# kyprifog/ballista

Measured on AMD Instinct MI355X. Metric: tpch_q1_sf100_rows_per_sec, higher is better.
Workload: dtype f64; 1 GPU; TPC-H Q1 SF100 (scan+filter+group-by aggregate), 600037902 lineitem rows resident in HBM, Arrow layout, Int32 order keys; lineitem_rows=600037902, rows_per_gpu=600037902, partitioning=1 GPU, whole tables

## Files before the change

ballista_amd/csrc/host/sop.cpp:

```cpp
#include "sop.hpp"

#include <cmath>
#include <cstring>
#include <limits>

namespace bhip {

namespace {

struct Builder {
    const Schema& schema;
    SopPlan& out;
    Builder(const Schema& s, SopPlan& o) : schema(s), out(o) {}

    int column(int schema_idx) {
        for (size_t i = 0; i < out.col_map.size(); ++i)
            if (out.col_map[i] == schema_idx) return (int)i;
        if ((int)out.col_map.size() >= SOP_NCOL) return -1;
        out.col_map.push_back(schema_idx);
        return (int)out.col_map.size() - 1;
    }

    int plain_column(const ExprPtr& e) const {
        if (e->kind != BHIP_EXPR_COLUMN) return -1;
        return schema.index_of(e->name);
    }

    bool predicate(const ExprPtr& e) {
        if (e->kind == BHIP_EXPR_BINARY && e->name == "And") return predicate(e->args[0]) && predicate(e->args[1]);
        if (e->kind != BHIP_EXPR_BINARY) return false;
        static const char* ops[] = {"Eq", "Lt", "LtEq", "Gt", "GtEq"};
        static const int flipped[] = {0, 3, 4, 1, 2};
        int k = -1;
        for (int i = 0; i < 5; ++i)
            if (e->name == ops[i]) k = i;
        if (k < 0) return false;
        ExprPtr colside = e->args[0], litside = e->args[1];
        if (colside->kind == BHIP_EXPR_LITERAL) { std::swap(colside, litside); k = flipped[k]; }
        const int ci = plain_column(colside);
        if (ci < 0) return false;
        const int t = schema.fields[ci].dtype;
        if (litside->kind != BHIP_EXPR_LITERAL || litside->is_null || litside->dtype != t) return false;
        double lit;
        bool is_int;
        if (t == DT_FLOAT64) { lit = litside->f64; is_int = false; }
        else if (t == DT_INT32 || t == DT_DATE32) { lit = (double)litside->i64; is_int = true; }
        else return false;
        if (std::isnan(lit)) return false;
        const double inf = std::numeric_limits<double>::infinity();
        double lo = -inf, hi = inf;
        switch (k) {
            case 0: lo = hi = lit; break;
            case 1: hi = is_int ? lit - 1.0 : std::nextafter(lit, -inf); break;
            case 2: hi = lit; break;
            case 3: lo = is_int ? lit + 1.0 : std::nextafter(lit, inf); break;
            default: lo = lit; break;
        }
        const int c = column(ci);
        if (c < 0) return false;
        for (int i = 0; i < out.prog.n_ranges; ++i)
            if (out.prog.ranges[i].col == c) {
                if (lo > out.prog.ranges[i].lo) out.prog.ranges[i].lo = lo;
                if (hi < out.prog.ranges[i].hi) out.prog.ranges[i].hi = hi;
                return true;
            }
        if (out.prog.n_ranges >= SOP_NRANGE) return false;
        SopRange& r = out.prog.ranges[out.prog.n_ranges++];
        memset(&r, 0, sizeof(r));
        r.col = (uint8_t)c;
        r.is32 = is_int ? 1 : 0;
        r.lo = lo;
        r.hi = hi;
        return true;
    }

    struct Factor { bool has_col; bool is32; int schema_col; double sgn, add; std::string text; };

    bool f64_column(const ExprPtr& e, int& col, bool& is32) const {
        if (e->kind == BHIP_EXPR_CAST && e->dtype == DT_FLOAT64) {
            const int i = plain_column(e->args[0]);
            if (i < 0) return false;
            const int t = schema.fields[i].dtype;
            if (t != DT_INT32 && t != DT_DATE32) return false;
            col = i; is32 = true;
            return true;
        }
        const int i = plain_column(e);
        if (i < 0 || schema.fields[i].dtype != DT_FLOAT64) return false;
        col = i; is32 = false;
        return true;
    }

    static bool f64_literal(const ExprPtr& e, double& v) {
        if (e->kind != BHIP_EXPR_LITERAL || e->dtype != DT_FLOAT64 || e->is_null) return false;
        v = e->f64;
        return true;
    }

    bool factor(const ExprPtr& e, Factor& f) const {
        f.text = e->to_string();
        f.has_col = true; f.is32 = false; f.schema_col = -1; f.sgn = 1.0; f.add = -0.0;
        double lit;
        if (f64_literal(e, lit)) { f.has_col = false; f.sgn = 0.0; f.add = lit; return true; }
        if (f64_column(e, f.schema_col, f.is32)) return true;
        if (e->kind == BHIP_EXPR_BINARY && (e->name == "Plus" || e->name == "Minus")) {
            const bool plus = e->name == "Plus";
            if (f64_literal(e->args[0], lit) && f64_column(e->args[1], f.schema_col, f.is32)) {
                f.sgn = plus ? 1.0 : -1.0;
                f.add = lit;
                return true;
            }
            if (f64_literal(e->args[1], lit) && f64_column(e->args[0], f.schema_col, f.is32)) {
                f.sgn = 1.0;
                f.add = plus ? lit : -lit;
                return true;
            }
        }
        return false;
    }

    bool chain(const ExprPtr& e, std::vector<Factor>& fs) const {
        Factor f;
        if (factor(e, f)) { fs.push_back(f); return true; }
        if (e->kind == BHIP_EXPR_BINARY && e->name == "Multiply") {
            if (!chain(e->args[0], fs)) return false;
            if (!factor(e->args[1], f)) return false;
            fs.push_back(f);
            return true;
        }
        return false;
    }
};

}

bool build_sop(const Schema& schema, const ExprPtr& predicate, const std::vector<ExprPtr>& keys,
               const std::vector<SopAccExpr>& accs, SopPlan& out) {
    memset(&out.prog, 0, sizeof(out.prog));
    out.col_map.clear();
    out.key_info.clear();
    Builder b(schema, out);
    if (predicate && !b.predicate(predicate)) return false;
    for (int i = 0; i < out.prog.n_ranges; ++i)
        if (out.prog.ranges[i].lo > out.prog.ranges[i].hi) return false;
    if (keys.size() > (size_t)SOP_NKEY) return false;
    for (size_t i = 0; i < keys.size(); ++i) {
        const int si = b.plain_column(keys[i]);
        if (si < 0) return false;
        const int t = schema.fields[si].dtype;
        int kind, width;
        if (t == DT_INT32 || t == DT_DATE32) { kind = SOP_KEY_I32; width = 4; }
        else if (t == DT_INT64 || t == DT_UINT64) { kind = SOP_KEY_I64; width = 8; }
        else if (t == DT_UTF8) { kind = SOP_KEY_UTF8; width = 8; }
        else return false;
        if (keys.size() == 3 && i >= 1 && kind != SOP_KEY_I32) return false;
        const int c = b.column(si);
        if (c < 0) return false;
        SopKey& k = out.prog.keys[out.prog.n_keys++];
        k.col = (uint8_t)c;
        k.kind = (uint8_t)kind;
        k.pad[0] = k.pad[1] = 0;
        const int pos = i == 0 ? 0 : (i == 1 ? 8 : 12);
        out.key_info.push_back(ProgramBuilder::KeyInfo{pos, width, 0, t});
    }
    std::vector<std::string> last_chain;
    for (size_t a = 0; a < accs.size(); ++a) {
        if (accs[a].kind != ACC_SUM_F64) return false;
        std::vector<Builder::Factor> fs;
        if (!b.chain(accs[a].expr, fs)) return false;
        size_t common = 0;
        if (!last_chain.empty() && fs.size() > last_chain.size()) {
            common = last_chain.size();
            for (size_t i = 0; i < last_chain.size(); ++i)
                if (fs[i].text != last_chain[i]) { common = 0; break; }
        }
        for (size_t i = common; i < fs.size(); ++i) {
            if (out.prog.n_steps >= SOP_NSTEP) return false;
            SopStep& st = out.prog.steps[out.prog.n_steps++];
            memset(&st, 0, sizeof(st));
            st.has_col = fs[i].has_col ? 1 : 0;
            st.is32 = fs[i].is32 ? 1 : 0;
            st.start = i == 0 ? 1 : 0;
            st.acc = 0xFF;
            st.sgn = fs[i].sgn;
            st.add = fs[i].add;
            if (fs[i].has_col) {
                const int c = b.column(fs[i].schema_col);
                if (c < 0) return false;
                st.col = (uint8_t)c;
            }
        }
        out.prog.steps[out.prog.n_steps - 1].acc = (uint8_t)a;
        last_chain.clear();
        for (auto& f : fs) last_chain.push_back(f.text);
    }
    out.prog.n_cols = (int)out.col_map.size();
    return true;
}

bool sop_columns_bindable(const SopPlan& plan, const Batch& b, bool range_nulls_ok) {
    for (size_t i = 0; i < plan.col_map.size(); ++i) {
        if (!b.cols[plan.col_map[i]].validity) continue;
        bool ranged = false;
        for (int r = 0; r < plan.prog.n_ranges; ++r) ranged = ranged || plan.prog.ranges[r].col == (uint8_t)i;
        if (!(range_nulls_ok && ranged)) return false;
    }
    return true;
}

void bind_sop(SopPlan& plan, const Batch& b) {
    plan.prog.n_rows = b.n_rows;
    for (size_t i = 0; i < plan.col_map.size(); ++i) {
        const Column& c = b.cols[plan.col_map[i]];
        SopColumn& sc = plan.prog.cols[i];
        sc.data = c.data ? c.data->ptr() : nullptr;
        sc.offsets = c.offsets ? c.offsets->as<int32_t>() : nullptr;
        sc.validity = c.validity ? c.validity->as<uint64_t>() : nullptr;
        sc.dtype = c.dtype;
        sc.data_bytes = (int32_t)c.data_bytes;
        sc.width = c.utf8_width(b.n_rows);
        sc.pad = 0;
    }
}

bool lean_eligible(const SopProgram& prog) {
    if (prog.n_keys > 2) return false;
    for (int q = 0; q < prog.n_keys; ++q)
        if (prog.keys[q].kind != SOP_KEY_I32 && prog.keys[q].kind != SOP_KEY_UTF8) return false;
    for (int s = 0; s < prog.n_steps; ++s) {
        const SopStep& st = prog.steps[s];
        if (!st.has_col || st.is32) return false;
        if (st.sgn != 1.0 && st.sgn != -1.0) return false;
    }
    return true;
}

bool lean_bindable(const SopPlan& plan, const Batch& b) {
    for (int ci : plan.col_map) {
        const Column& c = b.cols[ci];
        if (c.data && ((uintptr_t)c.data->ptr() & 15)) return false;
        if (c.offsets && ((uintptr_t)c.offsets->ptr() & 15)) return false;
        if (c.dtype == DT_UTF8 && c.data && !c.data->owned()) return false;
    }
    return true;
}

}
```

ballista_amd/csrc/lean_kernel.h:

```cpp
#pragma once
#include <hip/hip_runtime.h>
#include "kernels.h"
#include "launch_common.h"
#include "reduce_device.h"
#include "sop.h"
#include "vm_device.h"

namespace bhip {

#ifndef LEAN_U_VALUE
#define LEAN_U_VALUE 2
#endif
constexpr int LEAN_U = LEAN_U_VALUE;
constexpr int LEAN_SUB = BLOCK * 2;
constexpr int LEAN_TILE = LEAN_SUB * LEAN_U;
constexpr int LEAN_ROWS = 2 * LEAN_U;
constexpr uint32_t LEAN_MAX_STR = 3;

template <int GMAX, int NSTEP>
struct LeanLds {
    static constexpr int NG = GMAX > 1 ? GMAX : 0;
    double acc[NG * NSTEP * BLOCK + 1];
    uint32_t cnt[NG * BLOCK + 1];
    uint64_t keys[AGG_GMAX];
    uint32_t ng, lock, overflow, pad;
    uint64_t red[4][GMAX * NSTEP];
    uint64_t rowred[4][GMAX];
    uint64_t rowtot[GMAX];
};

struct LeanU3 { uint32_t a, b, c; };
struct alignas(8) LeanU2 { uint32_t x, y; };
struct alignas(16) LeanU4 { uint32_t x, y, z, w; };

__device__ inline LeanU2 lean_ld2(const BHIP_GLOBAL char* p) {
    const BHIP_GLOBAL LeanU2* q = (const BHIP_GLOBAL LeanU2*)p;
    LeanU2 v;
    v.x = q->x; v.y = q->y;
    return v;
}
__device__ inline LeanU4 lean_ld4(const BHIP_GLOBAL char* p) {
    const BHIP_GLOBAL LeanU4* q = (const BHIP_GLOBAL LeanU4*)p;
    LeanU4 v;
    v.x = q->x; v.y = q->y; v.z = q->z; v.w = q->w;
    return v;
}

__device__ inline uint64_t lean_uniform_u64(uint64_t v) {
    const uint32_t lo = __builtin_amdgcn_readfirstlane((uint32_t)v), hi = __builtin_amdgcn_readfirstlane((uint32_t)(v >> 32));
    return ((uint64_t)hi << 32) | lo;
}

__device__ inline uint32_t lean_str_word(uint32_t raw, uint32_t len) {
    return (__builtin_amdgcn_ubfe(raw, 0u, len << 3) << 8) | len;
}

template <bool ON>
struct LeanLens {
    uint32_t any[2] = {0u, 0u};
    uint32_t all[2] = {~0u, ~0u};
    __device__ void see(int q, uint32_t len) { any[q] |= len; all[q] &= len; }
};
template <>
struct LeanLens<false> {
    uint32_t bad = 0;
    __device__ void see(int, uint32_t len) { bad |= len; }
};

template <int GMAX, int NSTEP>
struct LeanKeyTable {
    int ng_c = 0;
    uint64_t gk[GMAX];
    __device__ LeanKeyTable() {
#pragma unroll
        for (int g = 0; g < GMAX; ++g) gk[g] = 0;
    }
    __device__ bool lookup(LeanLds<GMAX, NSTEP>& lds, int lane, const uint64_t (&key)[LEAN_ROWS], const bool (&live)[LEAN_ROWS],
                           int (&lg)[LEAN_ROWS]) {
        if constexpr (GMAX == 1) {
#pragma unroll
            for (int r = 0; r < LEAN_ROWS; ++r) lg[r] = live[r] ? 0 : -1;
            return true;
        } else {
            volatile uint32_t* v_ng = &lds.ng;
            volatile uint32_t* v_over = &lds.overflow;
            for (;;) {
                bool pending = false;
#pragma unroll
                for (int r = 0; r < LEAN_ROWS; ++r) {
                    int found = -2;
#pragma unroll
                    for (int g2 = 0; g2 < GMAX; ++g2) found = (g2 < ng_c && key[r] == gk[g2]) ? g2 : found;
                    lg[r] = live[r] ? found : -1;
                    pending |= (lg[r] == -2);
                }
                const uint64_t pmask = __ballot(pending);
                if (__builtin_expect(pmask == 0, 1)) return true;
                if (__builtin_amdgcn_readfirstlane(*v_over)) return false;
                if (__builtin_amdgcn_readfirstlane(*v_ng) == (uint32_t)ng_c) {
                    if (lane == (int)__builtin_ctzll(pmask)) {
                        uint64_t mine = 0;
#pragma unroll
                        for (int r = LEAN_ROWS - 1; r >= 0; --r)
                            if (lg[r] == -2) mine = key[r];
                        while (atomicCAS(&lds.lock, 0u, 1u) != 0u) {}
                        const int n2 = (int)*v_ng;
                        bool have = false;
                        for (int g2 = 0; g2 < n2; ++g2) have |= (lds.keys[g2] == mine);
                        if (!have) {
                            if (n2 < GMAX) {
                                lds.keys[n2] = mine;
                                __threadfence_block();
                                *v_ng = (uint32_t)(n2 + 1);
                            } else {
                                *v_over = 1;
                            }
                        }
                        __threadfence_block();
                        atomicExch(&lds.lock, 0u);
                    }
                }
                ng_c = __builtin_amdgcn_readfirstlane((int)*v_ng);
#pragma unroll
                for (int g2 = 0; g2 < GMAX; ++g2) gk[g2] = lean_uniform_u64(lds.keys[g2]);
            }
        }
    }
};

template <int GMAX, int NSTEP, int NRANGE, class Lens, class Lookup, class Accumulate>
__device__ inline bool lean_tail(const SopProgram& S, int64_t tail0, int64_t n_rows, Lens& lens, Lookup&& lookup,
                                 Accumulate&& accumulate) {
    constexpr int NKEY = 2;
    const int tid = threadIdx.x;
    for (int k = 0; k < LEAN_TILE / BLOCK; ++k) {
        const int64_t i = tail0 + (int64_t)k * BLOCK + tid;
        const bool in = i < n_rows;
        bool ok = in;
        uint32_t w[NKEY] = {0, 0};
        double tv[NSTEP];
#pragma unroll
        for (int s = 0; s < NSTEP; ++s) tv[s] = 0.0;
        if (in) {
#pragma unroll
            for (int p = 0; p < NRANGE; ++p)
                if (p < S.n_ranges) {
                    const SopRange rg = S.ranges[p];
                    const BHIP_GLOBAL char* base = (const BHIP_GLOBAL char*)S.cols[rg.col].data;
                    const double x = rg.is32 ? (double)*(const BHIP_GLOBAL int32_t*)(base + i * 4) : *(const BHIP_GLOBAL double*)(base + i * 8);
                    ok = ok && x >= rg.lo && x <= rg.hi;
                    const BHIP_GLOBAL uint64_t* vb = (const BHIP_GLOBAL uint64_t*)S.cols[rg.col].validity;
                    if (vb) ok = ok && ((vb[i >> 6] >> (i & 63)) & 1ull);
                }
#pragma unroll
            for (int q = 0; q < NKEY; ++q)
                if (q < S.n_keys) {
                    const SopColumn c = S.cols[S.keys[q].col];
                    if (S.keys[q].kind == SOP_KEY_UTF8) {
                        const uint32_t o0 = (uint32_t)c.offsets[i];
                        uint32_t len = (uint32_t)c.offsets[i + 1] - o0;
                        lens.see(q, len);
                        len = len > LEAN_MAX_STR ? LEAN_MAX_STR : len;
                        w[q] = lean_str_word((uint32_t)((const BHIP_GLOBAL PackedU64*)((const BHIP_GLOBAL char*)c.data + o0))->v, len);
                    } else {
                        w[q] = *(const BHIP_GLOBAL uint32_t*)((const BHIP_GLOBAL char*)c.data + i * 4);
                    }
                }
#pragma unroll
            for (int s = 0; s < NSTEP; ++s)
                if (s < S.n_steps) {
                    const SopStep st = S.steps[s];
                    const bool plain = st.sgn == 1.0 && st.add == 0.0 && __builtin_signbit(st.add);
                    const uint32_t flip = st.sgn < 0.0 ? 0x80000000u : 0u;
                    const double x = *(const BHIP_GLOBAL double*)((const BHIP_GLOBAL char*)S.cols[st.col].data + i * 8);
                    const double f = plain ? x : u2d(d2u(x) ^ ((uint64_t)flip << 32)) + st.add;
                    tv[s] = (s > 0 && !st.start) ? tv[s - (s > 0)] * f : f;
                }
        }
        uint64_t key[LEAN_ROWS];
        bool live[LEAN_ROWS];
        int lg[LEAN_ROWS];
#pragma unroll
        for (int r = 0; r < LEAN_ROWS; ++r) { key[r] = 0; live[r] = false; }
        key[0] = ((uint64_t)w[1] << 32) | w[0];
        live[0] = ok;
        if (!lookup(key, live, lg)) return false;
        accumulate(lg[0], tv);
    }
    return true;
}

template <int GMAX, int NSTEP>
__device__ inline void lean_finish(LeanLds<GMAX, NSTEP>& lds, const SopProgram& S, const double (&acc)[NSTEP], uint32_t rows1,
                                   const LeanLens<(GMAX > 1)>& lens, GroupRec* partials, uint32_t* partial_ng, ScanStatus* status) {
    const int tid = threadIdx.x, lane = tid & 63, wave = tid >> 6;
    if constexpr (GMAX > 1) {
        uint32_t len_bits = 0;
#pragma unroll
        for (int q = 0; q < 2; ++q) {
            const uint32_t b = (lens.any[q] & 3u) | (lens.any[q] > LEAN_MAX_STR ? 4u : 0u) | ((~lens.all[q] & 3u) << 3);
            len_bits |= b << (SCAN_LEN_SHIFT + q * SCAN_LEN_BITS);
        }
        if (len_bits) atomicOr(&lds.pad, len_bits);
    }
    __syncthreads();
    uint64_t tot_rows = 0;
    double tot_acc = 0.0;
#pragma unroll
    for (int g = 0; g < GMAX; ++g) {
        const uint32_t mine = GMAX == 1 ? rows1 : lds.cnt[(GMAX > 1 ? g : 0) * BLOCK + tid];
        const uint64_t v = wave_reduce((uint64_t)mine, ACC_COUNT_ROWS);
        if (lane == 0) lds.rowred[wave][g] = v;
    }
#pragma unroll
    for (int g = 0; g < GMAX; ++g)
#pragma unroll
        for (int s = 0; s < NSTEP; ++s) {
            const double mine = GMAX == 1 ? acc[s] : lds.acc[(GMAX > 1 ? (g * NSTEP + s) : 0) * BLOCK + tid];
            const uint64_t v = wave_reduce(d2u(mine), ACC_SUM_F64);
            if (lane == 0) lds.red[wave][g * NSTEP + s] = v;
        }
    __syncthreads();
    if (tid < GMAX) {
        tot_rows = lds.rowred[0][tid] + lds.rowred[1][tid] + lds.rowred[2][tid] + lds.rowred[3][tid];
        lds.rowtot[tid] = tot_rows;
    }
    if (tid < GMAX * NSTEP)
        tot_acc = ((u2d(lds.red[0][tid]) + u2d(lds.red[1][tid])) + u2d(lds.red[2][tid])) + u2d(lds.red[3][tid]);
    __syncthreads();

    GroupRec* out = partials + (size_t)blockIdx.x * GMAX;
    if (tid < GMAX) {
        out[tid].k0 = lds.keys[tid] & 0xFFFFFFFFull;
        out[tid].k1 = lds.keys[tid] >> 32;
        out[tid].rows = tot_rows;
    }
    if (tid < GMAX * NSTEP) {
        const int g = tid / NSTEP, s = tid % NSTEP;
        if (s < S.n_steps && S.steps[s].acc != 0xFF) {
            out[g].acc[S.steps[s].acc] = d2u(tot_acc);
            out[g].nvalid[S.steps[s].acc] = lds.rowtot[g];
        }
    }
    if (tid == 0) {
        partial_ng[blockIdx.x] = GMAX == 1 ? (tot_rows > 0 ? 1u : 0u) : lds.ng;
        if constexpr (GMAX > 1) {
            const uint32_t lb = lds.pad;
            const bool too_long = (lb & ((4u << SCAN_LEN_SHIFT) | (4u << (SCAN_LEN_SHIFT + SCAN_LEN_BITS)))) != 0;
            const uint32_t f = lb | (lds.overflow ? (uint32_t)SCAN_OVERFLOW_GROUPS : 0u) | (too_long ? (uint32_t)SCAN_ERR_KEY_TOO_LONG : 0u);
            if (f) atomicOr(&status->flags, f);
        } else {
            if (lds.overflow) atomicOr(&status->flags, SCAN_OVERFLOW_GROUPS);
        }
    }
    if constexpr (GMAX == 1) {
        if (lens.bad > LEAN_MAX_STR) atomicOr(&status->flags, SCAN_ERR_KEY_TOO_LONG);
    }
}

template <int GMAX, int NSTEP, int NRANGE>
__global__ void __launch_bounds__(BLOCK, (GMAX == 1 && NSTEP <= 5) ? 4 : 3)
scan_agg_lean_kernel(const SopProgram* __restrict__ Sp, GroupRec* partials, uint32_t* partial_ng, ScanStatus* status) {
    const SopProgram& S = *Sp;
    constexpr int U = LEAN_U;
    constexpr int NKEY = 2;
    __shared__ LeanLds<GMAX, NSTEP> lds;
    const int tid = threadIdx.x, lane = tid & 63;

    const int n_ranges = S.n_ranges, n_keys = S.n_keys, n_steps = S.n_steps;
    const int64_t n_rows = S.n_rows;
    const int64_t n_tiles = n_rows / LEAN_TILE;
    const int64_t grid = gridDim.x;
    const int64_t row0 = (int64_t)blockIdx.x * LEAN_TILE;
    const int64_t stride = grid * LEAN_TILE;

    const BHIP_GLOBAL char* rp[NRANGE];
    const BHIP_GLOBAL uint64_t* rvp[NRANGE];
    bool r32[NRANGE];
    double rlo[NRANGE], rhi[NRANGE];
#pragma unroll
    for (int p = 0; p < NRANGE; ++p) {
        rp[p] = nullptr; rvp[p] = nullptr; r32[p] = false; rlo[p] = -__builtin_huge_val(); rhi[p] = __builtin_huge_val();
        if (p < n_ranges) {
            r32[p] = S.ranges[p].is32 != 0;
            rp[p] = (const BHIP_GLOBAL char*)S.cols[S.ranges[p].col].data + row0 * (r32[p] ? 4 : 8);
            if (S.cols[S.ranges[p].col].validity) rvp[p] = (const BHIP_GLOBAL uint64_t*)S.cols[S.ranges[p].col].validity + row0 / 64;
            rlo[p] = S.ranges[p].lo; rhi[p] = S.ranges[p].hi;
        }
    }
    const BHIP_GLOBAL char* kp[NKEY];
    const BHIP_GLOBAL char* kdat[NKEY];
    bool kutf[NKEY];
#pragma unroll
    for (int q = 0; q < NKEY; ++q) {
        kp[q] = nullptr; kdat[q] = nullptr; kutf[q] = false;
        if (q < n_keys) {
            const SopColumn c = S.cols[S.keys[q].col];
            kutf[q] = S.keys[q].kind == SOP_KEY_UTF8;
            kp[q] = (kutf[q] ? (const BHIP_GLOBAL char*)c.offsets : (const BHIP_GLOBAL char*)c.data) + row0 * 4;
            kdat[q] = (const BHIP_GLOBAL char*)c.data;
        }
    }
    const BHIP_GLOBAL char* xp[NSTEP];
    bool xstart[NSTEP], xplain[NSTEP];
    uint32_t xflip[NSTEP];
    double xadd[NSTEP];
#pragma unroll
    for (int s = 0; s < NSTEP; ++s) {
        xp[s] = nullptr; xstart[s] = true; xplain[s] = true; xflip[s] = 0; xadd[s] = 0.0;
        if (s < n_steps) {
            const SopStep st = S.steps[s];
            xstart[s] = st.start != 0;
            xplain[s] = st.sgn == 1.0 && st.add == 0.0 && __builtin_signbit(st.add);
            xflip[s] = st.sgn < 0.0 ? 0x80000000u : 0u;
            xadd[s] = st.add;
            xp[s] = (const BHIP_GLOBAL char*)S.cols[st.col].data + row0 * 8;
        }
    }

    double acc[NSTEP];
    uint32_t rows1 = 0;
#pragma unroll
    for (int s = 0; s < NSTEP; ++s) acc[s] = 0.0;
    if constexpr (GMAX > 1) {
#pragma unroll
        for (int j = 0; j < GMAX * NSTEP; ++j) lds.acc[j * BLOCK + tid] = 0.0;
#pragma unroll
        for (int j = 0; j < GMAX; ++j) lds.cnt[j * BLOCK + tid] = 0;
    }
    if (tid == 0) { lds.ng = 0; lds.overflow = 0; lds.lock = 0; }
    if (GMAX > 1 && tid == 0) lds.pad = 0;
    if (tid < AGG_GMAX) lds.keys[tid] = 0;
    __syncthreads();
    LeanLens<(GMAX > 1)> lens;
    LeanKeyTable<GMAX, NSTEP> table;
    auto lookup = [&](const uint64_t (&key)[LEAN_ROWS], const bool (&live)[LEAN_ROWS], int (&lg)[LEAN_ROWS]) -> bool {
        return table.lookup(lds, lane, key, live, lg);
    };
    auto accumulate = [&](int lgr, const double (&tv)[NSTEP]) {
        if constexpr (GMAX == 1) {
            if (lgr >= 0) {
                rows1 += 1;
#pragma unroll
                for (int s = 0; s < NSTEP; ++s) acc[s] += tv[s];
            }
        } else {
            if (lgr >= 0) {
                double* a = &lds.acc[lgr * (NSTEP * BLOCK) + tid];
#pragma unroll
                for (int s = 0; s < NSTEP; ++s)
                    __hip_atomic_fetch_add(a + s * BLOCK, tv[s], __ATOMIC_RELAXED, __HIP_MEMORY_SCOPE_WORKGROUP);
                __hip_atomic_fetch_add(&lds.cnt[lgr * BLOCK + tid], 1u, __ATOMIC_RELAXED, __HIP_MEMORY_SCOPE_WORKGROUP);
            }
        }
    };

    LeanU4 rv[NRANGE][U];
    uint64_t rvw[NRANGE][U];
    uint32_t kv[NKEY][U][2];
    uint64_t kb[NKEY][U];
    LeanU3 ko[NKEY][U];
    LeanU4 xv[NSTEP][U];
#pragma unroll
    for (int u = 0; u < U; ++u) {
#pragma unroll
        for (int p = 0; p < NRANGE; ++p) { rv[p][u] = LeanU4{0, 0, 0, 0}; rvw[p][u] = ~0ull; }
#pragma unroll
        for (int q = 0; q < NKEY; ++q) { kv[q][u][0] = kv[q][u][1] = 0; kb[q][u] = 0; ko[q][u] = LeanU3{0, 0, 0}; }
#pragma unroll
        for (int s = 0; s < NSTEP; ++s) xv[s][u] = LeanU4{0, 0, 0, 0};
    }
    const uint32_t t8 = (uint32_t)tid * 8u, t16 = (uint32_t)tid * 16u;

    auto load_ranges = [&]() {
#pragma unroll
        for (int p = 0; p < NRANGE; ++p)
            if (p < n_ranges) {
                if (r32[p]) {
#pragma unroll
                    for (int u = 0; u < U; ++u) {
                        const LeanU2 v = lean_ld2(rp[p] + u * (LEAN_SUB * 4) + t8);
                        rv[p][u].x = v.x; rv[p][u].y = v.y;
                    }
                } else {
#pragma unroll
                    for (int u = 0; u < U; ++u) rv[p][u] = lean_ld4(rp[p] + u * (LEAN_SUB * 8) + t16);
                }
                if (rvp[p]) {
#pragma unroll
                    for (int u = 0; u < U; ++u) rvw[p][u] = rvp[p][u * (LEAN_SUB / 64) + (tid >> 5)];
                }
            }
    };
    auto load_offsets = [&]() {
#pragma unroll
        for (int q = 0; q < NKEY; ++q)
            if (q < n_keys && kutf[q]) {
#pragma unroll
                for (int u = 0; u < U; ++u) {
                    const BHIP_GLOBAL char* a = kp[q] + u * (LEAN_SUB * 4) + t8;
                    const LeanU2 v = lean_ld2(a);
                    ko[q][u].a = v.x; ko[q][u].b = v.y;
                    ko[q][u].c = *(const BHIP_GLOBAL uint32_t*)(a + 8);
                }
            }
    };
    auto load_keys = [&]() {
#pragma unroll
        for (int q = 0; q < NKEY; ++q)
            if (q < n_keys) {
                if (kutf[q]) {
#pragma unroll
                    for (int u = 0; u < U; ++u) {
                        const uint32_t l0 = ko[q][u].b - ko[q][u].a, l1 = ko[q][u].c - ko[q][u].b;
                        lens.see(q, l0); lens.see(q, l1);
                        kv[q][u][0] = l0; kv[q][u][1] = l1;
                        kb[q][u] = ((const BHIP_GLOBAL PackedU64*)(kdat[q] + ko[q][u].a))->v;
                    }
                } else {
#pragma unroll
                    for (int u = 0; u < U; ++u) {
                        const LeanU2 v = lean_ld2(kp[q] + u * (LEAN_SUB * 4) + t8);
                        kv[q][u][0] = v.x; kv[q][u][1] = v.y;
                    }
                }
            }
    };
    auto load_steps = [&]() {
#pragma unroll
        for (int s = 0; s < NSTEP; ++s)
            if (s < n_steps) {
#pragma unroll
                for (int u = 0; u < U; ++u) xv[s][u] = lean_ld4(xp[s] + u * (LEAN_SUB * 8) + t16);
            }
    };
    auto advance_keys_utf8 = [&]() {
#pragma unroll
        for (int q = 0; q < NKEY; ++q)
            if (kutf[q]) kp[q] += stride * 4;
    };
    auto advance_rest = [&]() {
#pragma unroll
        for (int p = 0; p < NRANGE; ++p) {
            rp[p] += stride * (r32[p] ? 4 : 8);
            if (rvp[p]) rvp[p] += stride / 64;
        }
#pragma unroll
        for (int q = 0; q < NKEY; ++q)
            if (!kutf[q]) kp[q] += stride * 4;
#pragma unroll
        for (int s = 0; s < NSTEP; ++s) xp[s] += stride * 8;
    };

    auto eval_live = [&](bool (&live)[LEAN_ROWS]) {
#pragma unroll
        for (int r = 0; r < LEAN_ROWS; ++r) live[r] = true;
#pragma unroll
        for (int p = 0; p < NRANGE; ++p)
            if (p < n_ranges) {
                if (r32[p]) {
#pragma unroll
                    for (int u = 0; u < U; ++u) {
                        const double a = (double)(int32_t)rv[p][u].x, b = (double)(int32_t)rv[p][u].y;
                        live[2 * u] = live[2 * u] && a >= rlo[p] && a <= rhi[p];
                        live[2 * u + 1] = live[2 * u + 1] && b >= rlo[p] && b <= rhi[p];
                    }
                } else {
#pragma unroll
                    for (int u = 0; u < U; ++u) {
                        const double a = u2d(((uint64_t)rv[p][u].y << 32) | rv[p][u].x), b = u2d(((uint64_t)rv[p][u].w << 32) | rv[p][u].z);
                        live[2 * u] = live[2 * u] && a >= rlo[p] && a <= rhi[p];
                        live[2 * u + 1] = live[2 * u + 1] && b >= rlo[p] && b <= rhi[p];
                    }
                }
                if (rvp[p]) {
                    const uint32_t bit = (2u * (uint32_t)tid) & 63u;
#pragma unroll
                    for (int u = 0; u < U; ++u) {
                        live[2 * u] = live[2 * u] && ((rvw[p][u] >> bit) & 1ull);
                        live[2 * u + 1] = live[2 * u + 1] && ((rvw[p][u] >> (bit + 1u)) & 1ull);
                    }
                }
            }
    };
    auto eval_keys = [&](uint64_t (&key)[LEAN_ROWS]) {
        uint32_t w[NKEY][LEAN_ROWS];
#pragma unroll
        for (int q = 0; q < NKEY; ++q) {
#pragma unroll
            for (int r = 0; r < LEAN_ROWS; ++r) w[q][r] = 0;
            if (q < n_keys) {
                if (kutf[q]) {
#pragma unroll
                    for (int u = 0; u < U; ++u) {
                        const uint32_t l0 = kv[q][u][0] > LEAN_MAX_STR ? LEAN_MAX_STR : kv[q][u][0];
                        const uint32_t l1 = kv[q][u][1] > LEAN_MAX_STR ? LEAN_MAX_STR : kv[q][u][1];
                        w[q][2 * u] = lean_str_word((uint32_t)kb[q][u], l0);
                        w[q][2 * u + 1] = lean_str_word((uint32_t)(kb[q][u] >> (l0 << 3)), l1);
                    }
                } else {
#pragma unroll
                    for (int u = 0; u < U; ++u) { w[q][2 * u] = kv[q][u][0]; w[q][2 * u + 1] = kv[q][u][1]; }
                }
            }
        }
#pragma unroll
        for (int r = 0; r < LEAN_ROWS; ++r) key[r] = ((uint64_t)w[1][r] << 32) | w[0][r];
    };
    auto eval_chain = [&]() {
#pragma unroll
        for (int s = 0; s < NSTEP; ++s)
            if (s < n_steps) {
                if (!xplain[s]) {
#pragma unroll
                    for (int u = 0; u < U; ++u) {
                        const double a = u2d(((uint64_t)(xv[s][u].y ^ xflip[s]) << 32) | xv[s][u].x) + xadd[s];
                        const double b = u2d(((uint64_t)(xv[s][u].w ^ xflip[s]) << 32) | xv[s][u].z) + xadd[s];
                        xv[s][u].x = (uint32_t)d2u(a); xv[s][u].y = (uint32_t)(d2u(a) >> 32);
                        xv[s][u].z = (uint32_t)d2u(b); xv[s][u].w = (uint32_t)(d2u(b) >> 32);
                    }
                }
                if (s > 0 && !xstart[s]) {
#pragma unroll
                    for (int u = 0; u < U; ++u) {
                        const double a = u2d(((uint64_t)xv[s - (s > 0)][u].y << 32) | xv[s - (s > 0)][u].x) * u2d(((uint64_t)xv[s][u].y << 32) | xv[s][u].x);
                        const double b = u2d(((uint64_t)xv[s - (s > 0)][u].w << 32) | xv[s - (s > 0)][u].z) * u2d(((uint64_t)xv[s][u].w << 32) | xv[s][u].z);
                        xv[s][u].x = (uint32_t)d2u(a); xv[s][u].y = (uint32_t)(d2u(a) >> 32);
                        xv[s][u].z = (uint32_t)d2u(b); xv[s][u].w = (uint32_t)(d2u(b) >> 32);
                    }
                }
            }
    };

    bool over = false;
    if ((int64_t)blockIdx.x < n_tiles) {
        load_offsets();
        load_ranges();
        load_steps();
        load_keys();
        advance_keys_utf8();
        if ((int64_t)blockIdx.x + grid < n_tiles) load_offsets();
        advance_keys_utf8();
    }
    for (int64_t t = blockIdx.x; t < n_tiles; t += grid) {
        const bool more1 = t + grid < n_tiles, more2 = t + 2 * grid < n_tiles;
        advance_rest();

        bool live[LEAN_ROWS];
        eval_live(live);
        if (more1) load_ranges();

        uint64_t key[LEAN_ROWS];
        eval_keys(key);
        if (more1) load_keys();
        if (more2) load_offsets();
        advance_keys_utf8();

        int lg[LEAN_ROWS];
        if (!lookup(key, live, lg)) { over = true; break; }

        eval_chain();
#pragma unroll
        for (int u = 0; u < U; ++u) {
            double ta[NSTEP], tb[NSTEP];
#pragma unroll
            for (int s = 0; s < NSTEP; ++s) {
                ta[s] = u2d(((uint64_t)xv[s][u].y << 32) | xv[s][u].x);
                tb[s] = u2d(((uint64_t)xv[s][u].w << 32) | xv[s][u].z);
            }
            accumulate(lg[2 * u], ta);
            accumulate(lg[2 * u + 1], tb);
        }
        if (more1) load_steps();
    }

    if (!over && (int64_t)blockIdx.x == n_tiles % grid && n_tiles * LEAN_TILE < n_rows)
        over = !lean_tail<GMAX, NSTEP, NRANGE>(S, n_tiles * LEAN_TILE, n_rows, lens, lookup, accumulate);

    lean_finish<GMAX, NSTEP>(lds, S, acc, rows1, lens, partials, partial_ng, status);
}

template <int GMAX>
static hipError_t launch_lean_g(const LaunchCfg& cfg, const SopProgram& S, SopProgram* dprog, GroupRec* partials,
                                uint32_t* partial_ng, int max_grid, ScanStatus* status, int* grid_out) {
#define BHIP_LEAN(NS_, NR_) launch_sop_program(scan_agg_lean_kernel<GMAX, NS_, NR_>, LEAN_TILE, cfg, S, dprog, partials, partial_ng, max_grid, status, grid_out)
    const bool few = S.n_ranges <= 1;
    if (S.n_steps <= 2) return few ? BHIP_LEAN(2, 1) : BHIP_LEAN(2, 4);
    if (S.n_steps <= 5) return few ? BHIP_LEAN(5, 1) : BHIP_LEAN(5, 4);
    return few ? BHIP_LEAN(8, 1) : BHIP_LEAN(8, 4);
#undef BHIP_LEAN
}

}
```

ballista_amd/csrc/sop.h:

```cpp
#pragma once
#include <hip/hip_runtime.h>
#include <stdint.h>
#include "kernels.h"

namespace bhip {

constexpr int SOP_NRANGE = 4;
constexpr int SOP_NKEY = 3;
constexpr int SOP_NSTEP = 8;
constexpr int SOP_NCOL = 16;

struct SopColumn {
    const void* data;
    const int32_t* offsets;
    const uint64_t* validity;
    int32_t dtype;
    int32_t data_bytes;
    int32_t width;
    int32_t pad;
};

struct SopRange {
    uint8_t col;
    uint8_t is32;
    uint8_t pad[6];
    double lo, hi;
};

struct SopStep {
    uint8_t col;
    uint8_t is32;
    uint8_t has_col;
    uint8_t start;
    uint8_t acc;
    uint8_t pad[3];
    double sgn, add;
};

enum SopKeyKind : uint8_t { SOP_KEY_I32 = 0, SOP_KEY_I64 = 1, SOP_KEY_UTF8 = 2 };
struct SopKey {
    uint8_t col;
    uint8_t kind;
    uint8_t pad[2];
};

struct SopProgram {
    int64_t n_rows;
    int32_t n_cols, n_ranges, n_keys, n_steps;
    SopColumn cols[SOP_NCOL];
    SopRange ranges[SOP_NRANGE];
    SopKey keys[SOP_NKEY];
    SopStep steps[SOP_NSTEP];
};

hipError_t launch_scan_agg_sop(const LaunchCfg& cfg, const SopProgram& S, SopProgram* dprog, int gmax, GroupRec* partials,
                               uint32_t* partial_ng, int max_grid, ScanStatus* status, int* grid_out);

hipError_t launch_scan_agg_lean(const LaunchCfg& cfg, const SopProgram& S, SopProgram* dprog, int gmax, GroupRec* partials,
                                uint32_t* partial_ng, int max_grid, ScanStatus* status, int* grid_out, const char** variant = nullptr,
                                bool* fixed_keys = nullptr);

hipError_t launch_range_bitmap(const LaunchCfg& cfg, const SopProgram& S, SopProgram* dprog, uint64_t* bitmap, uint32_t* tile_counts);
struct Utf8Literal { uint8_t bytes[64]; int32_t len; };
hipError_t launch_utf8_eq_bitmap(const LaunchCfg& cfg, const int32_t* offsets, const void* data, const uint64_t* validity, int64_t n, const Utf8Literal& lit,
                                 bool negate, uint64_t* bitmap, uint32_t* tile_counts);

}
```

Measured before the change: 154.9 billion rows/s.

## Skip step-column loads for rows failing range filter, prefetch ranges two tiles ahead

```diff
diff --git a/ballista_amd/csrc/host/sop.cpp b/ballista_amd/csrc/host/sop.cpp
--- a/ballista_amd/csrc/host/sop.cpp
+++ b/ballista_amd/csrc/host/sop.cpp
@@ -195,6 +195,8 @@
         for (auto& f : fs) last_chain.push_back(f.text);
     }
     out.prog.n_cols = (int)out.col_map.size();
+    static const bool no_masked_loads = env_flag("BHIP_NO_MASKED_LOADS");
+    out.prog.dense_loads = no_masked_loads ? 1 : 0;
     return true;
 }
 
diff --git a/ballista_amd/csrc/lean_kernel.h b/ballista_amd/csrc/lean_kernel.h
--- a/ballista_amd/csrc/lean_kernel.h
+++ b/ballista_amd/csrc/lean_kernel.h
@@ -45,6 +45,11 @@
     v.x = q->x; v.y = q->y; v.z = q->z; v.w = q->w;
     return v;
 }
+
+typedef uint32_t LeanV2 __attribute__((ext_vector_type(2)));
+typedef uint32_t LeanV4 __attribute__((ext_vector_type(4)));
+__device__ inline LeanV2 lean_ldv2(const BHIP_GLOBAL char* p) { return *(const BHIP_GLOBAL LeanV2*)p; }
+__device__ inline LeanV4 lean_ldv4(const BHIP_GLOBAL char* p) { return *(const BHIP_GLOBAL LeanV4*)p; }
 
 __device__ inline uint64_t lean_uniform_u64(uint64_t v) {
     const uint32_t lo = __builtin_amdgcn_readfirstlane((uint32_t)v), hi = __builtin_amdgcn_readfirstlane((uint32_t)(v >> 32));
@@ -267,7 +272,8 @@
     __shared__ LeanLds<GMAX, NSTEP> lds;
     const int tid = threadIdx.x, lane = tid & 63;
 
-    const int n_ranges = S.n_ranges, n_keys = S.n_keys, n_steps = S.n_steps;
+    const int n_ranges = S.n_ranges, n_keys = GMAX > 1 ? S.n_keys : 0, n_steps = S.n_steps;
+    const bool dense = S.dense_loads != 0;
     const int64_t n_rows = S.n_rows;
     const int64_t n_tiles = n_rows / LEAN_TILE;
     const int64_t grid = gridDim.x;
@@ -355,20 +361,21 @@
         }
     };
 
-    LeanU4 rv[NRANGE][U];
+    LeanV2 rv32[NRANGE][U];
+    LeanV4 rv64[NRANGE][U];
     uint64_t rvw[NRANGE][U];
     uint32_t kv[NKEY][U][2];
     uint64_t kb[NKEY][U];
     LeanU3 ko[NKEY][U];
-    LeanU4 xv[NSTEP][U];
+    LeanV4 xv[NSTEP][U];
 #pragma unroll
     for (int u = 0; u < U; ++u) {
 #pragma unroll
-        for (int p = 0; p < NRANGE; ++p) { rv[p][u] = LeanU4{0, 0, 0, 0}; rvw[p][u] = ~0ull; }
+        for (int p = 0; p < NRANGE; ++p) { rv32[p][u] = LeanV2{0, 0}; rv64[p][u] = LeanV4{0, 0, 0, 0}; rvw[p][u] = ~0ull; }
 #pragma unroll
         for (int q = 0; q < NKEY; ++q) { kv[q][u][0] = kv[q][u][1] = 0; kb[q][u] = 0; ko[q][u] = LeanU3{0, 0, 0}; }
 #pragma unroll
-        for (int s = 0; s < NSTEP; ++s) xv[s][u] = LeanU4{0, 0, 0, 0};
+        for (int s = 0; s < NSTEP; ++s) xv[s][u] = LeanV4{0, 0, 0, 0};
     }
     const uint32_t t8 = (uint32_t)tid * 8u, t16 = (uint32_t)tid * 16u;
 
@@ -378,13 +385,10 @@
             if (p < n_ranges) {
                 if (r32[p]) {
 #pragma unroll
-                    for (int u = 0; u < U; ++u) {
-                        const LeanU2 v = lean_ld2(rp[p] + u * (LEAN_SUB * 4) + t8);
-                        rv[p][u].x = v.x; rv[p][u].y = v.y;
-                    }
+                    for (int u = 0; u < U; ++u) rv32[p][u] = lean_ldv2(rp[p] + u * (LEAN_SUB * 4) + t8);
                 } else {
 #pragma unroll
-                    for (int u = 0; u < U; ++u) rv[p][u] = lean_ld4(rp[p] + u * (LEAN_SUB * 8) + t16);
+                    for (int u = 0; u < U; ++u) rv64[p][u] = lean_ldv4(rp[p] + u * (LEAN_SUB * 8) + t16);
                 }
                 if (rvp[p]) {
 #pragma unroll
@@ -426,12 +430,14 @@
                 }
             }
     };
-    auto load_steps = [&]() {
-#pragma unroll
-        for (int s = 0; s < NSTEP; ++s)
-            if (s < n_steps) {
-#pragma unroll
-                for (int u = 0; u < U; ++u) xv[s][u] = lean_ld4(xp[s] + u * (LEAN_SUB * 8) + t16);
+    auto load_steps = [&](uint32_t lv) {
+        if (dense) lv = ~0u;
+#pragma unroll
+        for (int u = 0; u < U; ++u)
+            if ((lv >> (2 * u)) & 3u) {
+#pragma unroll
+                for (int s = 0; s < NSTEP; ++s)
+                    if (s < n_steps) xv[s][u] = lean_ldv4(xp[s] + u * (LEAN_SUB * 8) + t16);
             }
     };
     auto advance_keys_utf8 = [&]() {
@@ -439,12 +445,14 @@
         for (int q = 0; q < NKEY; ++q)
             if (kutf[q]) kp[q] += stride * 4;
     };
-    auto advance_rest = [&]() {
+    auto advance_ranges = [&]() {
 #pragma unroll
         for (int p = 0; p < NRANGE; ++p) {
             rp[p] += stride * (r32[p] ? 4 : 8);
             if (rvp[p]) rvp[p] += stride / 64;
         }
+    };
+    auto advance_rest = [&]() {
 #pragma unroll
         for (int q = 0; q < NKEY; ++q)
             if (!kutf[q]) kp[q] += stride * 4;
@@ -452,7 +460,8 @@
         for (int s = 0; s < NSTEP; ++s) xp[s] += stride * 8;
     };
 
-    auto eval_live = [&](bool (&live)[LEAN_ROWS]) {
+    auto eval_live = [&]() -> uint32_t {
+        bool live[LEAN_ROWS];
 #pragma unroll
         for (int r = 0; r < LEAN_ROWS; ++r) live[r] = true;
 #pragma unroll
@@ -461,14 +470,14 @@
                 if (r32[p]) {
 #pragma unroll
                     for (int u = 0; u < U; ++u) {
-                        const double a = (double)(int32_t)rv[p][u].x, b = (double)(int32_t)rv[p][u].y;
+                        const double a = (double)(int32_t)rv32[p][u].x, b = (double)(int32_t)rv32[p][u].y;
                         live[2 * u] = live[2 * u] && a >= rlo[p] && a <= rhi[p];
                         live[2 * u + 1] = live[2 * u + 1] && b >= rlo[p] && b <= rhi[p];
                     }
                 } else {
 #pragma unroll
                     for (int u = 0; u < U; ++u) {
-                        const double a = u2d(((uint64_t)rv[p][u].y << 32) | rv[p][u].x), b = u2d(((uint64_t)rv[p][u].w << 32) | rv[p][u].z);
+                        const double a = u2d(((uint64_t)rv64[p][u].y << 32) | rv64[p][u].x), b = u2d(((uint64_t)rv64[p][u].w << 32) | rv64[p][u].z);
                         live[2 * u] = live[2 * u] && a >= rlo[p] && a <= rhi[p];
                         live[2 * u + 1] = live[2 * u + 1] && b >= rlo[p] && b <= rhi[p];
                     }
@@ -482,6 +491,10 @@
                     }
                 }
             }
+        uint32_t lv = 0;
+#pragma unroll
+        for (int r = 0; r < LEAN_ROWS; ++r) lv |= live[r] ? (1u << r) : 0u;
+        return lv;
     };
     auto eval_keys = [&](uint64_t (&key)[LEAN_ROWS]) {
         uint32_t w[NKEY][LEAN_ROWS];
@@ -533,22 +546,28 @@
     };
 
     bool over = false;
+    uint32_t lv = 0;
     if ((int64_t)blockIdx.x < n_tiles) {
+        const bool more1 = (int64_t)blockIdx.x + grid < n_tiles;
         load_offsets();
         load_ranges();
-        load_steps();
+        advance_ranges();
         load_keys();
         advance_keys_utf8();
-        if ((int64_t)blockIdx.x + grid < n_tiles) load_offsets();
+        if (more1) load_offsets();
         advance_keys_utf8();
+        lv = eval_live();
+        load_steps(lv);
+        if (more1) load_ranges();
+        advance_ranges();
     }
     for (int64_t t = blockIdx.x; t < n_tiles; t += grid) {
         const bool more1 = t + grid < n_tiles, more2 = t + 2 * grid < n_tiles;
         advance_rest();
 
         bool live[LEAN_ROWS];
-        eval_live(live);
-        if (more1) load_ranges();
+#pragma unroll
+        for (int r = 0; r < LEAN_ROWS; ++r) live[r] = (lv >> r) & 1u;
 
         uint64_t key[LEAN_ROWS];
         eval_keys(key);
@@ -571,7 +590,12 @@
             accumulate(lg[2 * u], ta);
             accumulate(lg[2 * u + 1], tb);
         }
-        if (more1) load_steps();
+        if (more1) {
+            lv = eval_live();
+            load_steps(lv);
+        }
+        if (more2) load_ranges();
+        advance_ranges();
     }
 
     if (!over && (int64_t)blockIdx.x == n_tiles % grid && n_tiles * LEAN_TILE < n_rows)
diff --git a/ballista_amd/csrc/sop.h b/ballista_amd/csrc/sop.h
--- a/ballista_amd/csrc/sop.h
+++ b/ballista_amd/csrc/sop.h
@@ -51,6 +51,8 @@
     SopRange ranges[SOP_NRANGE];
     SopKey keys[SOP_NKEY];
     SopStep steps[SOP_NSTEP];
+    int32_t dense_loads;
+    int32_t pad;
 };
 
 hipError_t launch_scan_agg_sop(const LaunchCfg& cfg, const SopProgram& S, SopProgram* dprog, int gmax, GroupRec* partials,
```

Result: no change. 155.7 billion rows/s, median of 4 (+0.6%).
